# JonasFrey96/Visual-Odom-Pipeline

Measured on AMD Instinct MI355X. Metric: frames/sec @1241x376, 2000 KLT pts, 10-frame BA window, higher is better.
Workload: dtype u8/i32 (KLT, Shi-Tomasi) + f64 (DLT, BA); 1 GPU; kitti_shaped_1241x376_2000pts_ba10; sequences_per_gpu=256, batched_contexts_per_gpu=1, distinct_image_sequences=8, tracked_points=jittered grid (SURVEY 8d's fallback), launch=plain, solves_stopped_by_cap=0, solves_cut_and_rerun=0

## Files before the change

visual-odom-pipeline_amd/csrc/vo_frame.hip:

```cpp
#include "vo_internal.h"

#include <stdlib.h>
#include <string.h>

#include <new>

__device__ __forceinline__ int d_reflect101(int p, int len) {
  if (len == 1) return 0;
  while (p < 0 || p >= len) p = (p < 0) ? -p : 2 * (len - 1) - p;
  return p;
}

struct bil_args {
  int maxk;
  signed char dx[49], dy[49];
  float sw[49];
};

__global__ void __launch_bounds__(256) k_pad_level0_bilateral(const uint8_t* __restrict__ raw, size_t raw_seq_stride,
                                                              const int32_t* __restrict__ frame_idx, int w, int h,
                                                              uint8_t* __restrict__ dst, size_t dst_seq_stride, int pitch,
                                                              int ph, bil_args A, const float* __restrict__ color_w) {
  __shared__ float s_cw[256];
  s_cw[threadIdx.x] = color_w[threadIdx.x];
  __syncthreads();
  const int X = blockIdx.x * blockDim.x + threadIdx.x;
  const int Y = blockIdx.y;
  if (X >= w + 2 * VO_PAD || Y >= ph) return;
  raw += (size_t)blockIdx.z * raw_seq_stride;
  dst += (size_t)blockIdx.z * dst_seq_stride;
  if (frame_idx) raw += (size_t)(*frame_idx) * w * h;
  const int x = d_reflect101(X - VO_PAD, w), y = d_reflect101(Y - VO_PAD, h);
  const int val0 = raw[(size_t)y * w + x];
  float sum = 0.f, wsum = 0.f;
  for (int k = 0; k < A.maxk; k++) {
    const int val = raw[(size_t)d_reflect101(y + A.dy[k], h) * w + d_reflect101(x + A.dx[k], w)];
    const int ad = val > val0 ? val - val0 : val0 - val;
    const float wt = A.sw[k] * s_cw[ad];
    sum += (float)val * wt;
    wsum += wt;
  }
  dst[(size_t)Y * pitch + X] = (uint8_t)(int)__builtin_rintf(sum / wsum);
}

__device__ __forceinline__ bool vo_split_index(unsigned gid, int rows, int gpr, int g_lo, int g_hi, int& Y, int& G) {
  const int gi = g_hi - g_lo, gb = gpr - gi;
  const unsigned n_int = (unsigned)rows * (unsigned)gi;
  if (gid < n_int) {
    Y = (int)(gid / (unsigned)gi);
    G = g_lo + (int)(gid - (unsigned)Y * (unsigned)gi);
    return true;
  }
  gid -= n_int;
  Y = gb > 0 ? (int)(gid / (unsigned)gb) : rows;
  const int j = gb > 0 ? (int)(gid - (unsigned)Y * (unsigned)gb) : 0;
  G = j < g_lo ? j : g_hi + (j - g_lo);
  return false;
}

__global__ void __launch_bounds__(256) k_pad_level0(const uint8_t* __restrict__ raw, size_t raw_seq_stride,
                                                    const int32_t* __restrict__ frame_idx, int w, int h,
                                                    uint8_t* __restrict__ dst, size_t dst_seq_stride, int pitch, int ph, int remap) {
  int blk, bseq;
  vo_xcd_assign(blockIdx.z * gridDim.x + blockIdx.x, gridDim.x, remap, blk, bseq);
  const int gpr = (w + 2 * VO_PAD + 15) / 16;
  const unsigned gid = (unsigned)blk * blockDim.x + threadIdx.x;
  const int g_lo = VO_PAD / 16, g_hi = max(g_lo, min(gpr, (w + VO_PAD - 16 >= 0 ? (w + VO_PAD - 16) / 16 + 1 : 0)));
  int Y, G;
  const bool interior = vo_split_index(gid, ph, gpr, g_lo, g_hi, Y, G);
  const int X = G * 16;
  if (Y >= ph) return;
  raw += (size_t)bseq * raw_seq_stride;
  dst += (size_t)bseq * dst_seq_stride;
  if (frame_idx) raw += (size_t)(*frame_idx) * w * h;
  const int y = d_reflect101(Y - VO_PAD, h);
  const uint8_t* row = raw + (size_t)y * w;
  uint32_t v[4];
  if (interior) {
    __builtin_memcpy(v, row + (X - VO_PAD), 16);
  } else {
#pragma unroll
    for (int q = 0; q < 4; q++) {
      v[q] = 0;
#pragma unroll
      for (int k = 0; k < 4; k++) v[q] |= (uint32_t)row[d_reflect101(X + 4 * q + k - VO_PAD, w)] << (8 * k);
    }
  }
  uint4 pk; pk.x = v[0]; pk.y = v[1]; pk.z = v[2]; pk.w = v[3];
  *reinterpret_cast<uint4*>(dst + (size_t)Y * pitch + X) = pk;
}

__device__ __forceinline__ int d_byte(uint32_t v, int k) { return (int)((v >> (8 * k)) & 0xFFu); }

__global__ void __launch_bounds__(256) k_scharr_pyrdown(const uint8_t* __restrict__ src, size_t src_seq_px, int w, int h, int pitch,
                                                        int16_t* __restrict__ der, int nb_scharr,
                                                        uint8_t* __restrict__ dst, size_t dst_seq_px, int dw, int dh, int dpitch, int remap) {
  int bx, bseq;
  vo_xcd_assign(blockIdx.y * gridDim.x + blockIdx.x, gridDim.x, remap, bx, bseq);
  src += (size_t)bseq * src_seq_px;
  if (bx < nb_scharr) {
    constexpr int SR = 4;
    const int gpr = (w + 3) / 4;
    const unsigned gid = (unsigned)bx * 256u + threadIdx.x;
    const int ys = (int)(gid / (unsigned)gpr);
    const int x0 = (int)(gid - (unsigned)ys * (unsigned)gpr) * 4;
    const int y0 = ys * SR;
    if (y0 >= h) return;
    typedef unsigned short u16x2 __attribute__((ext_vector_type(2)));
    typedef short s16x2 __attribute__((ext_vector_type(2)));
    auto load_row = [&](int yy, u16x2 (&a)[3]) {
      const uint32_t* q = reinterpret_cast<const uint32_t*>(src + (size_t)(yy + VO_PAD) * pitch + (x0 + VO_PAD));
      const uint32_t L = q[-1], M = q[0], R = q[1];
      a[0] = __builtin_bit_cast(u16x2, __builtin_amdgcn_perm(M, L, 0x0c040c03u));
      a[1] = __builtin_bit_cast(u16x2, __builtin_amdgcn_perm(0u, M, 0x0c020c01u));
      a[2] = __builtin_bit_cast(u16x2, __builtin_amdgcn_perm(R, M, 0x0c040c03u));
    };
    u16x2 rows[SR + 2][3];
#pragma unroll
    for (int r = 0; r < SR + 2; r++) load_row(min(y0 - 1 + r, h), rows[r]);
#pragma unroll
    for (int r = 0; r < SR; r++) {
      const int y = y0 + r;
      if (y >= h) break;
      s16x2 cs[3], dv[3];
#pragma unroll
      for (int c = 0; c < 3; c++) {
        cs[c] = __builtin_bit_cast(s16x2, (u16x2)((rows[r][c] + rows[r + 2][c]) * (unsigned short)12 + rows[r + 1][c] * (unsigned short)40));
        dv[c] = __builtin_bit_cast(s16x2, (u16x2)(rows[r + 2][c] - rows[r][c]));
      }
      const uint32_t ix01 = __builtin_bit_cast(uint32_t, (s16x2)(cs[1] - cs[0]));
      const uint32_t ix23 = __builtin_bit_cast(uint32_t, (s16x2)(cs[2] - cs[1]));
      const s16x2 w_lo = {12, 40}, w_hi = {40, 12}, w_0 = {12, 0}, w_1 = {0, 12};
      const int iy0 = __builtin_amdgcn_sdot2(dv[1], w_0, __builtin_amdgcn_sdot2(dv[0], w_lo, 0, false), false);
      const int iy1 = __builtin_amdgcn_sdot2(dv[1], w_hi, __builtin_amdgcn_sdot2(dv[0], w_1, 0, false), false);
      const int iy2 = __builtin_amdgcn_sdot2(dv[2], w_0, __builtin_amdgcn_sdot2(dv[1], w_lo, 0, false), false);
      const int iy3 = __builtin_amdgcn_sdot2(dv[2], w_hi, __builtin_amdgcn_sdot2(dv[1], w_1, 0, false), false);
      uint32_t out[4];
      out[0] = __builtin_amdgcn_perm((uint32_t)iy0, ix01, 0x05040100u);
      out[1] = __builtin_amdgcn_perm((uint32_t)iy1, ix01, 0x05040302u);
      out[2] = __builtin_amdgcn_perm((uint32_t)iy2, ix23, 0x05040100u);
      out[3] = __builtin_amdgcn_perm((uint32_t)iy3, ix23, 0x05040302u);
      if (x0 + 3 >= w) {
#pragma unroll
        for (int k = 1; k < 4; k++) if (x0 + k >= w) out[k] = 0u;
      }
      uint4 pk; pk.x = out[0]; pk.y = out[1]; pk.z = out[2]; pk.w = out[3];
      const size_t o = (size_t)(y + VO_PAD) * pitch + (x0 + VO_PAD);
      *reinterpret_cast<uint4*>(reinterpret_cast<uint32_t*>(der) + (size_t)bseq * src_seq_px + o) = pk;
    }
  } else {
    const int b = bx - nb_scharr;
    const int pw = dw + 2 * VO_PAD;
    const int gpr = (pw + 3) / 4;
    const unsigned gid = (unsigned)b * 256u + threadIdx.x;
    const int g_lo = VO_PAD / 4, g_hi = max(g_lo, min(gpr, (dw + VO_PAD - 4 >= 0 ? (dw + VO_PAD - 4) / 4 + 1 : 0)));
    int Y, G;
    const bool interior = vo_split_index(gid, dh + 2 * VO_PAD, gpr, g_lo, g_hi, Y, G);
    const int X0 = G * 4;
    if (Y >= dh + 2 * VO_PAD) return;
    const int y = d_reflect101(Y - VO_PAD, dh);
    const uint8_t* prow = src + (size_t)(2 * y + VO_PAD) * pitch + VO_PAD;
    uint32_t res = 0;
    if (interior) {
      const int x0 = X0 - VO_PAD;
      uint32_t acc[4] = {128u, 128u, 128u, 128u};
#pragma unroll
      for (int j = -2; j <= 2; j++) {
        const uint32_t* q = reinterpret_cast<const uint32_t*>(prow + (ptrdiff_t)j * pitch + 2 * x0);
        const uint32_t d0 = q[-1], d1 = q[0], d2 = q[1], d3 = q[2];
        const uint32_t wj = (j == 0) ? 6u : ((j == -1 || j == 1) ? 4u : 1u);
        acc[0] = __builtin_amdgcn_udot4(d1, wj * 0x00010406u, __builtin_amdgcn_udot4(d0, wj * 0x04010000u, acc[0], false), false);
        acc[1] = __builtin_amdgcn_udot4(d2, wj * 0x00000001u, __builtin_amdgcn_udot4(d1, wj * 0x04060401u, acc[1], false), false);
        acc[2] = __builtin_amdgcn_udot4(d2, wj * 0x00010406u, __builtin_amdgcn_udot4(d1, wj * 0x04010000u, acc[2], false), false);
        acc[3] = __builtin_amdgcn_udot4(d3, wj * 0x00000001u, __builtin_amdgcn_udot4(d2, wj * 0x04060401u, acc[3], false), false);
      }
      res = __builtin_amdgcn_perm(__builtin_amdgcn_perm(acc[3], acc[2], 0x0c0c0501u), __builtin_amdgcn_perm(acc[1], acc[0], 0x0c0c0501u), 0x05040100u);
    } else {
#pragma unroll
      for (int k = 0; k < 4; k++) {
        const int x = d_reflect101(X0 + k - VO_PAD, dw);
        const uint8_t* p = prow + 2 * x;
        int sum = 0;
#pragma unroll
        for (int j = -2; j <= 2; j++) {
          const uint8_t* r = p + (ptrdiff_t)j * pitch;
          const int row = r[-2] + 4 * r[-1] + 6 * r[0] + 4 * r[1] + r[2];
          const int wj = (j == 0) ? 6 : ((j == -1 || j == 1) ? 4 : 1);
          sum += wj * row;
        }
        res |= (uint32_t)((sum + 128) >> 8) << (8 * k);
      }
    }
    *reinterpret_cast<uint32_t*>(dst + (size_t)bseq * dst_seq_px + (size_t)Y * dpitch + X0) = res;
  }
}

static hipEvent_t prof_event(vo_ctx* c) {
  vo_prof& p = c->prof;
  if (p.used == p.pool.size()) {
    hipEvent_t e = nullptr;
    if (hipEventCreate(&e) != hipSuccess) return nullptr;
    p.pool.push_back(e);
  }
  return p.pool[p.used++];
}

vo_prof_scope::vo_prof_scope(vo_ctx* c_, hipStream_t q_, int region_) : c(c_), q(q_), region(region_) {
  if (!((c->prof.mask >> region) & 1)) return;
  e0 = prof_event(c); e1 = prof_event(c);
  if (e0) (void)hipEventRecord(e0, q);
}

vo_prof_scope::~vo_prof_scope() {
  if (!e0 || !e1) return;
  (void)hipEventRecord(e1, q);
  c->prof.pairs[region].push_back(std::make_pair(e0, e1));
}

extern "C" int32_t vo_profile_enable(vo_ctx* c, int32_t region_mask) {
  if (!c) return VO_E_INVALID;
  VO_HIP(c, hipSetDevice(c->device));
  VO_HIP(c, hipStreamSynchronize(c->stream));
  c->prof.mask = region_mask;
  c->prof.used = 0;
  for (int r = 0; r < VO_PROF_COUNT; r++) c->prof.pairs[r].clear();
  return VO_OK;
}

extern "C" int32_t vo_debug_cycles(vo_ctx* c, int32_t which, int64_t* out8) {
  if (!c) return VO_E_INVALID;
  VO_CHECK(c, which >= 0 && which < 4 && out8, VO_E_INVALID, "bad selector");
  VO_HIP(c, hipSetDevice(c->device));
  VO_HIP(c, hipStreamSynchronize(c->stream));
  unsigned long long h[8];
  VO_HIP(c, hipMemcpy(h, c->d_dbg + 8 * which, sizeof(h), hipMemcpyDeviceToHost));
  out8[0] = 0;
  for (int i = 1; i < 8; i++) out8[i] = (h[i] && h[i - 1] && !(which == 0 && i >= 5)) ? (int64_t)(h[i] - h[i - 1]) : 0;
  for (int i = 1; i < 8; i++) out8[0] += out8[i];
  if (which == 0) { out8[7] = (int64_t)h[6]; out8[5] = (h[5] && h[2]) ? (int64_t)(h[5] - h[2]) : 0; }
  return VO_OK;
}

extern "C" int32_t vo_profile_read(vo_ctx* c, int32_t region, double* total_ms, int32_t* count) {
  if (!c) return VO_E_INVALID;
  VO_CHECK(c, region >= 0 && region < VO_PROF_COUNT && total_ms && count, VO_E_INVALID, "bad region");
  VO_HIP(c, hipSetDevice(c->device));
  VO_HIP(c, hipStreamSynchronize(c->stream));
  double t = 0;
  for (auto& pr : c->prof.pairs[region]) {
    float ms = 0;
    VO_HIP(c, hipEventElapsedTime(&ms, pr.first, pr.second));
    t += ms;
  }
  *total_ms = t; *count = (int32_t)c->prof.pairs[region].size();
  return VO_OK;
}

extern "C" int32_t vo_abi_version(void) { return VO_ABI_VERSION; }

bool vo_blocking_sync() {
  static const bool on = getenv("VO_BLOCKING_SYNC") && atoi(getenv("VO_BLOCKING_SYNC")) != 0;
  return on;
}

extern "C" int32_t vo_device_count(int32_t* n) {
  if (!n) return VO_E_INVALID;
  int c = 0;
  if (hipGetDeviceCount(&c) != hipSuccess) { *n = 0; return VO_E_HIP; }
  *n = c;
  return VO_OK;
}

static thread_local std::string g_create_err;

extern "C" const char* vo_last_error(const vo_ctx* ctx) {
  return ctx ? ctx->err.c_str() : g_create_err.c_str();
}

extern "C" int32_t vo_ctx_destroy(vo_ctx* c) {
  if (!c) return VO_OK;
  (void)hipSetDevice(c->device);
  if (c->stream) (void)hipStreamSynchronize(c->stream);
  if (c->stream2) (void)hipStreamSynchronize(c->stream2);
  if (c->stream_h2d) (void)hipStreamSynchronize(c->stream_h2d);
  if (c->stream3) (void)hipStreamSynchronize(c->stream3);
  (void)vo_comm_destroy(c);
  vo_pipe_destroy(c);
  vo_trk_destroy(c);
  vo_pnp_destroy(c);
  vo_ess_destroy(c);
  vo_hom_destroy(c);
  vo_fund_destroy(c);
  vo_hpose_destroy(c);
  vo_match_destroy(c);
  vo_sift_destroy(c);
  vo_st_destroy(c);
  vo_ba_destroy(c);
  vo_fb_destroy(c);
  vo_guess_destroy(c);
  vo_subpix_destroy(c);
  vo_brief_destroy(c);
  vo_orb_destroy(c);
  vo_ingest_free(&c->und_on, &c->d_und, (void**)&c->d_und_tab);
  vo_ingest_free(&c->cl_on, &c->d_clahe, (void**)&c->d_clahe_lut);
  for (int f = 0; f < 2; f++)
    for (int l = 0; l < VO_MAX_LEVELS; l++) {
      if (c->fr[f].img[l]) (void)hipFree(c->fr[f].img[l]);
      if (c->fr[f].der[l]) (void)hipFree(c->fr[f].der[l]);
    }
  for (auto& g : c->step_graphs) if (g.second) (void)hipGraphExecDestroy(g.second);
  void* bufs[] = {c->d_bil_cw, c->d_dbg, c->d_raw, c->d_seq, c->d_iters, c->d_uv0, c->d_uv1, c->d_slab, c->d_frame_idx, c->d_dlt_cam};
  for (void* b : bufs) if (b) (void)hipFree(b);
  if (c->h_slab) (void)hipHostFree(c->h_slab);
  if (c->h_frame_idx) (void)hipHostFree(c->h_frame_idx);
  if (c->h_raw) (void)hipHostFree(c->h_raw);
  if (c->ev_raw) (void)hipEventDestroy(c->ev_raw);
  for (hipEvent_t e : c->prof.pool) (void)hipEventDestroy(e);
  for (int k = 0; k < 2; k++) if (c->ev_step[k]) (void)hipEventDestroy(c->ev_step[k]);
  if (c->ev_fork) (void)hipEventDestroy(c->ev_fork);
  if (c->ev_join) (void)hipEventDestroy(c->ev_join);
  if (c->stream2) (void)hipStreamDestroy(c->stream2);
  if (c->stream3) (void)hipStreamDestroy(c->stream3);
  for (int k = 0; k < 2; k++) {
    if (c->d_host_raw[k]) (void)hipFree(c->d_host_raw[k]);
    if (c->ev_h2d[k]) (void)hipEventDestroy(c->ev_h2d[k]);
    if (c->ev_raw_free[k]) (void)hipEventDestroy(c->ev_raw_free[k]);
  }
  if (c->stream_h2d) (void)hipStreamDestroy(c->stream_h2d);
  if (c->h_ptr_tab) (void)hipHostFree(c->h_ptr_tab);
  for (int k = 0; k < 2; k++) if (c->ev_ba_wide[k]) (void)hipEventDestroy(c->ev_ba_wide[k]);
  for (int k = 0; k < 2; k++) { if (c->ev_ba[k]) (void)hipEventDestroy(c->ev_ba[k]); if (c->ev_pub[k]) (void)hipEventDestroy(c->ev_pub[k]); if (c->ev_copy1[k]) (void)hipEventDestroy(c->ev_copy1[k]); }
  if (c->stream) (void)hipStreamDestroy(c->stream);
  delete c;
  return VO_OK;
}

hipError_t vo_stream_create(hipStream_t* st, int reserve_cus) {
  int dev = 0, n_cu = 0;
  if (reserve_cus > 0 && (hipGetDevice(&dev) != hipSuccess || hipDeviceGetAttribute(&n_cu, hipDeviceAttributeMultiprocessorCount, dev) != hipSuccess)) n_cu = 0;
  if (reserve_cus <= 0 || n_cu <= 2 * reserve_cus || n_cu > 1024) return hipStreamCreateWithFlags(st, hipStreamNonBlocking);
  uint32_t mask[32];
  for (int k = 0; k < 32; k++) mask[k] = 0;
  for (int b = 0; b < n_cu - reserve_cus; b++) mask[b >> 5] |= 1u << (b & 31);
  return hipExtStreamCreateWithCUMask(st, (uint32_t)((n_cu + 31) / 32), mask);
}

extern "C" int32_t vo_ctx_create(int32_t device, int32_t width, int32_t height, int32_t max_pts,
                                 int32_t max_level, int32_t win, vo_ctx** out) {
  return vo_ctx_create_batched(device, width, height, max_pts, max_level, win, 1, out);
}

extern "C" int32_t vo_ctx_create_batched(int32_t device, int32_t width, int32_t height, int32_t max_pts,
                                         int32_t max_level, int32_t win, int32_t batch, vo_ctx** out) {
  if (!out) return VO_E_INVALID;
  *out = nullptr;
  if (width < 7 || height < 7 || max_pts < 1 || max_level < 0 || max_level >= VO_MAX_LEVELS ||
      win < 3 || win > VO_MAX_WIN || (win & 1) == 0 || batch < 1 || batch > 1024) {
    g_create_err = "vo_ctx_create: invalid argument";
    return VO_E_INVALID;
  }
  int ndev = 0;
  if (hipGetDeviceCount(&ndev) != hipSuccess || ndev <= 0) {
    g_create_err = "vo_ctx_create: no HIP device (this library has no CPU fallback)";
    return VO_E_HIP;
  }
  if (device < 0 || device >= ndev) { g_create_err = "vo_ctx_create: bad device index"; return VO_E_INVALID; }
  vo_ctx* c = new (std::nothrow) vo_ctx();
  if (!c) return VO_E_NOMEM;
  for (int f = 0; f < 2; f++)
    for (int l = 0; l < VO_MAX_LEVELS; l++) { c->fr[f].img[l] = nullptr; c->fr[f].der[l] = nullptr; }
  c->device = device; c->width = width; c->height = height; c->max_pts = max_pts; c->batch = batch;
  c->max_level = max_level; c->win = win;
  auto fail = [&](int32_t code) { g_create_err = c->err; vo_ctx_destroy(c); return code; };
#define CR(expr) do { hipError_t _e = (expr); if (_e != hipSuccess) { c->err = std::string(#expr) + " -> " + hipGetErrorString(_e); return fail(VO_E_HIP); } } while (0)
  CR(hipSetDevice(device));
  CR(hipStreamCreateWithFlags(&c->stream, hipStreamNonBlocking));
  CR(hipStreamCreateWithFlags(&c->stream2, hipStreamNonBlocking));

  CR(hipEventCreateWithFlags(&c->ev_fork, hipEventDisableTiming));
  CR(hipEventCreateWithFlags(&c->ev_join, hipEventDisableTiming));
  {
    const unsigned fl = hipEventDisableTiming | (vo_blocking_sync() ? hipEventBlockingSync : 0u);
    CR(hipEventCreateWithFlags(&c->ev_step[0], fl));
    CR(hipEventCreateWithFlags(&c->ev_step[1], fl));
  }
  int w = width, h = height, top = 0;
  for (int l = 0; l <= max_level; l++) {
    if (l > 0) {
      const int nw = (w + 1) / 2, nh = (h + 1) / 2;
      if (nw <= win || nh <= win) break;
      w = nw; h = nh;
    }
    c->lv[l].w = w; c->lv[l].h = h;
    c->lv[l].pitch = ((w + 2 * VO_PAD + 63) / 64) * 64;
    c->lv[l].ph = h + 2 * VO_PAD;
    c->lvl_px[l] = (size_t)c->lv[l].pitch * c->lv[l].ph;
    top = l;
  }
  c->top = top;
  for (int f = 0; f < 2; f++)
    for (int l = 0; l <= top; l++) {
      const size_t px = c->lvl_px[l] * (size_t)batch;
      CR(hipMalloc((void**)&c->fr[f].img[l], px));
      CR(hipMalloc((void**)&c->fr[f].der[l], px * 4));
      CR(hipMemsetAsync(c->fr[f].img[l], 0, px, c->stream));
      CR(hipMemsetAsync(c->fr[f].der[l], 0, px * 4, c->stream));
    }
  CR(hipMalloc((void**)&c->d_raw, (size_t)width * height * batch));
  CR(hipMalloc((void**)&c->d_dbg, sizeof(unsigned long long) * 32));
  CR(hipMemsetAsync(c->d_dbg, 0, sizeof(unsigned long long) * 32, c->stream));
  {
    size_t off = 0;
    auto take = [&](size_t bytes) { const size_t o = off; off = (off + bytes + 255) & ~(size_t)255; return o; };
    const size_t M = (size_t)max_pts;
    c->off_pa = take(8 * M); c->off_pb = take(8 * M); c->off_status = take(M); c->off_err = take(4 * M);
    c->off_X4 = take(16 * M); c->off_depth = take(8 * M); c->off_reproj = take(8 * M);
    c->off_st_scalars = take(64); c->off_st_out = take(8 * 4096);
    c->slab_seq = off;
    c->slab_bytes = off * (size_t)batch;
    CR(hipMalloc((void**)&c->d_slab, c->slab_bytes));
    CR(hipMemsetAsync(c->d_slab, 0, c->slab_bytes, c->stream));
    CR(hipHostMalloc((void**)&c->h_slab, 2 * c->slab_bytes, hipHostMallocDefault));
  }
  CR(hipMalloc((void**)&c->d_iters, sizeof(int32_t) * (size_t)max_pts * VO_MAX_LEVELS * batch));
  CR(hipMalloc((void**)&c->d_uv0, sizeof(float) * 2 * (size_t)max_pts * batch));
  CR(hipMalloc((void**)&c->d_uv1, sizeof(float) * 2 * (size_t)max_pts * batch));
  CR(hipMalloc((void**)&c->d_frame_idx, sizeof(int32_t)));
  CR(hipHostMalloc((void**)&c->h_frame_idx, sizeof(int32_t) * 64, hipHostMallocDefault));
  CR(hipStreamSynchronize(c->stream));
#undef CR
  *out = c;
  return VO_OK;
}

extern "C" int32_t vo_sync(vo_ctx* c) {
  if (!c) return VO_E_INVALID;
  VO_HIP(c, hipSetDevice(c->device));
  { const int32_t rs = vo_sync_streams(c); if (rs != VO_OK) return rs; }
  if (c->stream_h2d) VO_HIP(c, hipStreamSynchronize(c->stream_h2d));
  return VO_OK;
}

int32_t vo_ingest_reserve(vo_ctx* c, uint8_t** staging) {
  if (!*staging) VO_HIP(c, hipMalloc((void**)staging, (size_t)c->width * c->height * c->batch));
  return VO_OK;
}

int32_t vo_ingest_commit(vo_ctx* c, bool* on) {
  VO_HIP(c, hipStreamSynchronize(c->stream));
  *on = true;
  c->ingest_gen++;
  return VO_OK;
}

void vo_ingest_free(bool* on, uint8_t** staging, void** table) {
  if (*staging) (void)hipFree(*staging);
  if (*table) (void)hipFree(*table);
  *staging = nullptr; *table = nullptr; *on = false;
}

int32_t vo_ingest_run(vo_ctx* c, const vo_ingest_stage& s, const char* off_msg, const uint8_t* img, int32_t stride, uint8_t* out) {
  VO_CHECK(c, img != nullptr && out != nullptr && stride >= c->width, VO_E_INVALID, "bad image / stride");
  VO_CHECK(c, s.on, VO_E_STATE, off_msg);
  VO_HIP(c, hipSetDevice(c->device));
  { const int32_t rq = vo_quiesce_side(c); if (rq != VO_OK) return rq; }
  const size_t rows = (size_t)c->height * c->batch, px = (size_t)c->width * c->height;
  VO_HIP(c, hipMemcpy2DAsync(c->d_raw, c->width, img, stride, c->width, rows, hipMemcpyHostToDevice, c->stream));
  s.enqueue(c, c->stream, c->d_raw, px, nullptr, 0);
  VO_HIP(c, hipGetLastError());
  VO_HIP(c, hipMemcpyAsync(out, s.staging, px * (size_t)c->batch, hipMemcpyDeviceToHost, c->stream));
  VO_HIP(c, hipStreamSynchronize(c->stream));
  return VO_OK;
}

int32_t vo_build_pyramid(vo_ctx* c, hipStream_t q, const uint8_t* d_raw_img, size_t raw_seq_stride, const int32_t* d_frame_idx) {
  vo_prof_scope prof(c, q, VO_PROF_FRAME);
  c->cur ^= 1;
  vo_frame& F = c->fr[c->cur];
  const int B = c->batch;
  const int remap = (!c->tune.xcd_remap_off && B % 8 == 0) ? 1 : 0;
  const vo_ingest_stage chain[2] = {{c->und_on, vo_undistort_enqueue, c->d_und}, {c->cl_on, vo_clahe_enqueue, c->d_clahe}};
  for (const vo_ingest_stage& s : chain)
    if (s.on) {
      s.enqueue(c, q, d_raw_img, raw_seq_stride, d_frame_idx, remap);
      d_raw_img = s.staging; raw_seq_stride = (size_t)c->width * c->height; d_frame_idx = nullptr;
    }
  {
    const vo_level& L = c->lv[0];
    dim3 grid(vo_div_up(((L.w + 2 * VO_PAD + 15) / 16) * L.ph, 256), 1, B);
    dim3 grid1(vo_div_up(L.w + 2 * VO_PAD, 256), L.ph, B);
    if (c->bil_maxk > 0) {
      bil_args A;
      A.maxk = c->bil_maxk;
      for (int k = 0; k < 49; k++) { A.dx[k] = c->bil_dx[k]; A.dy[k] = c->bil_dy[k]; A.sw[k] = c->bil_sw[k]; }
      hipLaunchKernelGGL(k_pad_level0_bilateral, grid1, dim3(256), 0, q, d_raw_img, raw_seq_stride, d_frame_idx, L.w,
                         L.h, F.img[0], c->lvl_px[0], L.pitch, L.ph, A, c->d_bil_cw);
    } else {
      hipLaunchKernelGGL(k_pad_level0, grid, dim3(256), 0, q, d_raw_img, raw_seq_stride, d_frame_idx, L.w, L.h,
                         F.img[0], c->lvl_px[0], L.pitch, L.ph, remap);
    }
  }
  for (int l = 0; l <= c->top; l++) {
    const vo_level& L = c->lv[l];
    const int nb_scharr = vo_div_up(vo_div_up(L.w, 4) * vo_div_up(L.h, 4), 256);
    int nb_down = 0;
    uint8_t* dst = nullptr; int dw = 0, dh = 0, dpitch = 0; size_t dpx = 0;
    if (l < c->top) {
      const vo_level& D = c->lv[l + 1];
      dst = F.img[l + 1]; dw = D.w; dh = D.h; dpitch = D.pitch; dpx = c->lvl_px[l + 1];
      nb_down = vo_div_up(vo_div_up(D.w + 2 * VO_PAD, 4) * D.ph, 256);
    }
    hipLaunchKernelGGL(k_scharr_pyrdown, dim3(nb_scharr + nb_down, B), dim3(256), 0, q,
                       F.img[l], c->lvl_px[l], L.w, L.h, L.pitch, F.der[l], nb_scharr, dst, dpx, dw, dh, dpitch, remap);
  }
  VO_HIP(c, hipGetLastError());
  c->n_pushed++;
  return VO_OK;
}

extern "C" int32_t vo_frame_push(vo_ctx* c, const uint8_t* img, int32_t stride) {
  if (!c) return VO_E_INVALID;
  VO_CHECK(c, img != nullptr && stride >= c->width, VO_E_INVALID, "bad image / stride");
  VO_HIP(c, hipSetDevice(c->device));
  { const int32_t rq = vo_quiesce_side(c); if (rq != VO_OK) return rq; }
  const size_t rows = (size_t)c->height * c->batch, bytes = rows * c->width;
  if (!c->h_raw) {
    VO_HIP(c, hipHostMalloc((void**)&c->h_raw, bytes, hipHostMallocDefault));
    VO_HIP(c, hipEventCreateWithFlags(&c->ev_raw, hipEventDisableTiming));
  } else {
    VO_HIP(c, hipEventSynchronize(c->ev_raw));
  }
  if (stride == c->width) memcpy(c->h_raw, img, bytes);
  else for (size_t y = 0; y < rows; y++) memcpy(c->h_raw + y * c->width, img + y * (size_t)stride, c->width);
  VO_HIP(c, hipMemcpyAsync(c->d_raw, c->h_raw, bytes, hipMemcpyHostToDevice, c->stream));
  VO_HIP(c, hipEventRecord(c->ev_raw, c->stream));
  return vo_build_pyramid(c, c->stream, c->d_raw, (size_t)c->width * c->height, nullptr);
}

extern "C" int32_t vo_seq_upload(vo_ctx* c, const uint8_t* frames, int32_t n_frames) {
  if (!c) return VO_E_INVALID;
  VO_CHECK(c, frames != nullptr && n_frames > 0, VO_E_INVALID, "bad sequence");
  VO_HIP(c, hipSetDevice(c->device));
  { const int32_t rs = vo_sync_streams(c); if (rs != VO_OK) return rs; }
  if (c->d_seq) { VO_HIP(c, hipFree(c->d_seq)); c->d_seq = nullptr; c->seq_n = 0; }
  const size_t bytes = (size_t)c->width * c->height * n_frames * c->batch;
  VO_HIP(c, hipMalloc((void**)&c->d_seq, bytes));
  VO_HIP(c, hipMemcpy(c->d_seq, frames, bytes, hipMemcpyHostToDevice));
  c->seq_n = n_frames;
  return VO_OK;
}

extern "C" int32_t vo_frame_push_resident(vo_ctx* c, int32_t idx) {
  if (!c) return VO_E_INVALID;
  VO_CHECK(c, c->d_seq != nullptr && idx >= 0 && idx < c->seq_n, VO_E_STATE, "no resident sequence / bad index");
  VO_HIP(c, hipSetDevice(c->device));
  { const int32_t rq = vo_quiesce_side(c); if (rq != VO_OK) return rq; }
  const size_t fr = (size_t)c->width * c->height;
  return vo_build_pyramid(c, c->stream, c->d_seq + (size_t)idx * fr, fr * c->seq_n, nullptr);
}

extern "C" int32_t vo_pyramid_level_size(vo_ctx* c, int32_t level, int32_t* w, int32_t* h) {
  if (!c) return VO_E_INVALID;
  VO_CHECK(c, level >= 0 && level <= c->top && w && h, VO_E_INVALID, "bad level");
  *w = c->lv[level].w; *h = c->lv[level].h;
  return VO_OK;
}

extern "C" int32_t vo_pyramid_read(vo_ctx* c, int32_t which, int32_t level, uint8_t* img_out, int16_t* deriv_out) {
  return vo_pyramid_read_seq(c, 0, which, level, img_out, deriv_out);
}

extern "C" int32_t vo_pyramid_read_seq(vo_ctx* c, int32_t seq, int32_t which, int32_t level, uint8_t* img_out, int16_t* deriv_out) {
  if (!c) return VO_E_INVALID;
  VO_CHECK(c, level >= 0 && level <= c->top && (which == 0 || which == 1) && seq >= 0 && seq < c->batch, VO_E_INVALID, "bad level / which / seq");
  VO_CHECK(c, c->n_pushed >= (which == 0 ? 2 : 1), VO_E_STATE, "frame not pushed yet");
  VO_HIP(c, hipSetDevice(c->device));
  const vo_frame& F = c->fr[which == 1 ? c->cur : (c->cur ^ 1)];
  const vo_level& L = c->lv[level];
  VO_HIP(c, hipStreamSynchronize(c->stream));
  if (img_out)
    VO_HIP(c, hipMemcpy2D(img_out, L.w, F.img[level] + (size_t)seq * c->lvl_px[level] + (size_t)VO_PAD * L.pitch + VO_PAD, L.pitch, L.w, L.h,
                          hipMemcpyDeviceToHost));
  if (deriv_out)
    VO_HIP(c, hipMemcpy2D(deriv_out, (size_t)L.w * 4, F.der[level] + ((size_t)seq * c->lvl_px[level] + (size_t)VO_PAD * L.pitch + VO_PAD) * 2,
                          (size_t)L.pitch * 4, (size_t)L.w * 4, L.h, hipMemcpyDeviceToHost));
  if (deriv_out)
    for (size_t i = 0, n = (size_t)L.w * L.h * 2; i < n; i++) deriv_out[i] = (int16_t)(deriv_out[i] / 4);
  return VO_OK;
}

extern "C" int32_t vo_set_prefilter(vo_ctx* c, int32_t d, double sigma_color, double sigma_space) {
  if (!c) return VO_E_INVALID;
  if (d == 0) { c->bil_maxk = 0; c->ingest_gen++; return VO_OK; }
  if (sigma_color <= 0) sigma_color = 1;
  if (sigma_space <= 0) sigma_space = 1;
  int radius = d < 0 ? (int)lrint(sigma_space * 1.5) : d / 2;
  if (radius < 1) radius = 1;
  VO_CHECK(c, radius <= 3, VO_E_CAPACITY, "bilateral pre-filter: diameter up to 7");
  VO_HIP(c, hipSetDevice(c->device));
  const double gc = -0.5 / (sigma_color * sigma_color), gs = -0.5 / (sigma_space * sigma_space);
  float cw[256];
  for (int i = 0; i < 256; i++) cw[i] = (float)exp((double)i * i * gc);
  int maxk = 0;
  for (int i = -radius; i <= radius; i++)
    for (int j = -radius; j <= radius; j++) {
      const double r = sqrt((double)i * i + (double)j * j);
      if (r > radius) continue;
      c->bil_sw[maxk] = (float)exp(r * r * gs);
      c->bil_dx[maxk] = (signed char)j; c->bil_dy[maxk] = (signed char)i;
      maxk++;
    }
  if (!c->d_bil_cw) VO_HIP(c, hipMalloc((void**)&c->d_bil_cw, sizeof(cw)));
  VO_HIP(c, hipMemcpyAsync(c->d_bil_cw, cw, sizeof(cw), hipMemcpyHostToDevice, c->stream));
  VO_HIP(c, hipStreamSynchronize(c->stream));
  c->bil_maxk = maxk;
  c->ingest_gen++;
  return VO_OK;
}
```

Measured before the change: 47720 frames/s.

## Walk row strips in Scharr and pyrDown with register rolling and prefetch

```diff
diff --git a/visual-odom-pipeline_amd/csrc/vo_frame.hip b/visual-odom-pipeline_amd/csrc/vo_frame.hip
--- a/visual-odom-pipeline_amd/csrc/vo_frame.hip
+++ b/visual-odom-pipeline_amd/csrc/vo_frame.hip
@@ -90,92 +90,168 @@
   *reinterpret_cast<uint4*>(dst + (size_t)Y * pitch + X) = pk;
 }
 
-__device__ __forceinline__ int d_byte(uint32_t v, int k) { return (int)((v >> (8 * k)) & 0xFFu); }
+constexpr int VO_WALK_ROWS = 4;
+
+constexpr int VO_SCHARR_STRIP = 8, VO_DOWN_STRIP = 2;
+
+__host__ __device__ inline void vo_down_groups(int dw, int& gpr, int& g_lo, int& g_hi) {
+  gpr = (dw + 2 * VO_PAD + 3) / 4;
+  g_lo = VO_PAD / 4;
+  const int hi = (dw + VO_PAD - 4 >= 0 ? (dw + VO_PAD - 4) / 4 + 1 : 0);
+  g_hi = g_lo > (gpr < hi ? gpr : hi) ? g_lo : (gpr < hi ? gpr : hi);
+}
 
 __global__ void __launch_bounds__(256) k_scharr_pyrdown(const uint8_t* __restrict__ src, size_t src_seq_px, int w, int h, int pitch,
-                                                        int16_t* __restrict__ der, int nb_scharr,
-                                                        uint8_t* __restrict__ dst, size_t dst_seq_px, int dw, int dh, int dpitch, int remap) {
+                                                        int16_t* __restrict__ der, int nb_scharr, int srows,
+                                                        uint8_t* __restrict__ dst, size_t dst_seq_px, int dw, int dh, int dpitch, int drows, int remap) {
   int bx, bseq;
   vo_xcd_assign(blockIdx.y * gridDim.x + blockIdx.x, gridDim.x, remap, bx, bseq);
   src += (size_t)bseq * src_seq_px;
+  typedef unsigned short u16x2 __attribute__((ext_vector_type(2)));
+  typedef short s16x2 __attribute__((ext_vector_type(2)));
+  typedef uint32_t u32x4 __attribute__((ext_vector_type(4)));
   if (bx < nb_scharr) {
-    constexpr int SR = 4;
+    constexpr int CH = VO_WALK_ROWS;
     const int gpr = (w + 3) / 4;
     const unsigned gid = (unsigned)bx * 256u + threadIdx.x;
     const int ys = (int)(gid / (unsigned)gpr);
     const int x0 = (int)(gid - (unsigned)ys * (unsigned)gpr) * 4;
-    const int y0 = ys * SR;
+    const int y0 = ys * srows;
     if (y0 >= h) return;
-    typedef unsigned short u16x2 __attribute__((ext_vector_type(2)));
-    typedef short s16x2 __attribute__((ext_vector_type(2)));
-    auto load_row = [&](int yy, u16x2 (&a)[3]) {
-      const uint32_t* q = reinterpret_cast<const uint32_t*>(src + (size_t)(yy + VO_PAD) * pitch + (x0 + VO_PAD));
-      const uint32_t L = q[-1], M = q[0], R = q[1];
-      a[0] = __builtin_bit_cast(u16x2, __builtin_amdgcn_perm(M, L, 0x0c040c03u));
-      a[1] = __builtin_bit_cast(u16x2, __builtin_amdgcn_perm(0u, M, 0x0c020c01u));
-      a[2] = __builtin_bit_cast(u16x2, __builtin_amdgcn_perm(R, M, 0x0c040c03u));
+    const int y1 = min(y0 + srows, h);
+    const uint8_t* col = src + (size_t)VO_PAD * pitch + (x0 + VO_PAD);
+    auto fetch = [&](int yy, uint32_t (&d)[3]) {
+      const uint32_t* q = reinterpret_cast<const uint32_t*>(col + (ptrdiff_t)min(yy, h) * pitch);
+      d[0] = q[-1]; d[1] = q[0]; d[2] = q[1];
     };
-    u16x2 rows[SR + 2][3];
-#pragma unroll
-    for (int r = 0; r < SR + 2; r++) load_row(min(y0 - 1 + r, h), rows[r]);
-#pragma unroll
-    for (int r = 0; r < SR; r++) {
-      const int y = y0 + r;
-      if (y >= h) break;
-      s16x2 cs[3], dv[3];
-#pragma unroll
-      for (int c = 0; c < 3; c++) {
-        cs[c] = __builtin_bit_cast(s16x2, (u16x2)((rows[r][c] + rows[r + 2][c]) * (unsigned short)12 + rows[r + 1][c] * (unsigned short)40));
-        dv[c] = __builtin_bit_cast(s16x2, (u16x2)(rows[r + 2][c] - rows[r][c]));
+    auto unpack = [&](const uint32_t (&d)[3], u16x2 (&a)[3]) {
+      a[0] = __builtin_bit_cast(u16x2, __builtin_amdgcn_perm(d[1], d[0], 0x0c040c03u));
+      a[1] = __builtin_bit_cast(u16x2, __builtin_amdgcn_perm(0u, d[1], 0x0c020c01u));
+      a[2] = __builtin_bit_cast(u16x2, __builtin_amdgcn_perm(d[2], d[1], 0x0c040c03u));
+    };
+    uint32_t raw[CH][3];
+    u16x2 rows[CH + 2][3];
+    {
+      uint32_t top[2][3];
+      fetch(y0 - 1, top[0]); fetch(y0, top[1]);
+#pragma unroll
+      for (int r = 0; r < CH; r++) fetch(y0 + 1 + r, raw[r]);
+      unpack(top[0], rows[0]); unpack(top[1], rows[1]);
+    }
+    uint32_t* out_px = reinterpret_cast<uint32_t*>(der) + (size_t)bseq * src_seq_px + (size_t)VO_PAD * pitch + (x0 + VO_PAD);
+    for (int y = y0; y < y1; y += CH) {
+#pragma unroll
+      for (int r = 0; r < CH; r++) unpack(raw[r], rows[r + 2]);
+      if (y + CH < y1) {
+#pragma unroll
+        for (int r = 0; r < CH; r++) fetch(y + CH + 1 + r, raw[r]);
       }
-      const uint32_t ix01 = __builtin_bit_cast(uint32_t, (s16x2)(cs[1] - cs[0]));
-      const uint32_t ix23 = __builtin_bit_cast(uint32_t, (s16x2)(cs[2] - cs[1]));
-      const s16x2 w_lo = {12, 40}, w_hi = {40, 12}, w_0 = {12, 0}, w_1 = {0, 12};
-      const int iy0 = __builtin_amdgcn_sdot2(dv[1], w_0, __builtin_amdgcn_sdot2(dv[0], w_lo, 0, false), false);
-      const int iy1 = __builtin_amdgcn_sdot2(dv[1], w_hi, __builtin_amdgcn_sdot2(dv[0], w_1, 0, false), false);
-      const int iy2 = __builtin_amdgcn_sdot2(dv[2], w_0, __builtin_amdgcn_sdot2(dv[1], w_lo, 0, false), false);
-      const int iy3 = __builtin_amdgcn_sdot2(dv[2], w_hi, __builtin_amdgcn_sdot2(dv[1], w_1, 0, false), false);
-      uint32_t out[4];
-      out[0] = __builtin_amdgcn_perm((uint32_t)iy0, ix01, 0x05040100u);
-      out[1] = __builtin_amdgcn_perm((uint32_t)iy1, ix01, 0x05040302u);
-      out[2] = __builtin_amdgcn_perm((uint32_t)iy2, ix23, 0x05040100u);
-      out[3] = __builtin_amdgcn_perm((uint32_t)iy3, ix23, 0x05040302u);
-      if (x0 + 3 >= w) {
-#pragma unroll
-        for (int k = 1; k < 4; k++) if (x0 + k >= w) out[k] = 0u;
+#pragma unroll
+      for (int r = 0; r < CH; r++) {
+        if (y + r >= y1) break;
+        s16x2 cs[3], dv[3];
+#pragma unroll
+        for (int c = 0; c < 3; c++) {
+          cs[c] = __builtin_bit_cast(s16x2, (u16x2)((rows[r][c] + rows[r + 2][c]) * (unsigned short)12 + rows[r + 1][c] * (unsigned short)40));
+          dv[c] = __builtin_bit_cast(s16x2, (u16x2)(rows[r + 2][c] - rows[r][c]));
+        }
+        const uint32_t ix01 = __builtin_bit_cast(uint32_t, (s16x2)(cs[1] - cs[0]));
+        const uint32_t ix23 = __builtin_bit_cast(uint32_t, (s16x2)(cs[2] - cs[1]));
+        const s16x2 w_lo = {12, 40}, w_hi = {40, 12}, w_0 = {12, 0}, w_1 = {0, 12};
+        const int iy0 = __builtin_amdgcn_sdot2(dv[1], w_0, __builtin_amdgcn_sdot2(dv[0], w_lo, 0, false), false);
+        const int iy1 = __builtin_amdgcn_sdot2(dv[1], w_hi, __builtin_amdgcn_sdot2(dv[0], w_1, 0, false), false);
+        const int iy2 = __builtin_amdgcn_sdot2(dv[2], w_0, __builtin_amdgcn_sdot2(dv[1], w_lo, 0, false), false);
+        const int iy3 = __builtin_amdgcn_sdot2(dv[2], w_hi, __builtin_amdgcn_sdot2(dv[1], w_1, 0, false), false);
+        uint32_t out[4];
+        out[0] = __builtin_amdgcn_perm((uint32_t)iy0, ix01, 0x05040100u);
+        out[1] = __builtin_amdgcn_perm((uint32_t)iy1, ix01, 0x05040302u);
+        out[2] = __builtin_amdgcn_perm((uint32_t)iy2, ix23, 0x05040100u);
+        out[3] = __builtin_amdgcn_perm((uint32_t)iy3, ix23, 0x05040302u);
+        if (x0 + 3 >= w) {
+#pragma unroll
+          for (int k = 1; k < 4; k++) if (x0 + k >= w) out[k] = 0u;
+        }
+        const u32x4 pk = {out[0], out[1], out[2], out[3]};
+        __builtin_nontemporal_store(pk, reinterpret_cast<u32x4*>(out_px + (size_t)(y + r) * pitch));
       }
-      uint4 pk; pk.x = out[0]; pk.y = out[1]; pk.z = out[2]; pk.w = out[3];
-      const size_t o = (size_t)(y + VO_PAD) * pitch + (x0 + VO_PAD);
-      *reinterpret_cast<uint4*>(reinterpret_cast<uint32_t*>(der) + (size_t)bseq * src_seq_px + o) = pk;
+#pragma unroll
+      for (int c = 0; c < 3; c++) { rows[0][c] = rows[CH][c]; rows[1][c] = rows[CH + 1][c]; }
     }
   } else {
     const int b = bx - nb_scharr;
-    const int pw = dw + 2 * VO_PAD;
-    const int gpr = (pw + 3) / 4;
-    const unsigned gid = (unsigned)b * 256u + threadIdx.x;
-    const int g_lo = VO_PAD / 4, g_hi = max(g_lo, min(gpr, (dw + VO_PAD - 4 >= 0 ? (dw + VO_PAD - 4) / 4 + 1 : 0)));
+    int gpr, g_lo, g_hi;
+    vo_down_groups(dw, gpr, g_lo, g_hi);
+    const int ph = dh + 2 * VO_PAD, nstrips = (dh + drows - 1) / drows;
+    unsigned gid = (unsigned)b * 256u + threadIdx.x;
+    const uint8_t* pcol = src + (size_t)VO_PAD * pitch + VO_PAD;
+    dst += (size_t)bseq * dst_seq_px;
     int Y, G;
-    const bool interior = vo_split_index(gid, dh + 2 * VO_PAD, gpr, g_lo, g_hi, Y, G);
-    const int X0 = G * 4;
-    if (Y >= dh + 2 * VO_PAD) return;
-    const int y = d_reflect101(Y - VO_PAD, dh);
-    const uint8_t* prow = src + (size_t)(2 * y + VO_PAD) * pitch + VO_PAD;
-    uint32_t res = 0;
-    if (interior) {
-      const int x0 = X0 - VO_PAD;
-      uint32_t acc[4] = {128u, 128u, 128u, 128u};
-#pragma unroll
-      for (int j = -2; j <= 2; j++) {
-        const uint32_t* q = reinterpret_cast<const uint32_t*>(prow + (ptrdiff_t)j * pitch + 2 * x0);
-        const uint32_t d0 = q[-1], d1 = q[0], d2 = q[1], d3 = q[2];
-        const uint32_t wj = (j == 0) ? 6u : ((j == -1 || j == 1) ? 4u : 1u);
-        acc[0] = __builtin_amdgcn_udot4(d1, wj * 0x00010406u, __builtin_amdgcn_udot4(d0, wj * 0x04010000u, acc[0], false), false);
-        acc[1] = __builtin_amdgcn_udot4(d2, wj * 0x00000001u, __builtin_amdgcn_udot4(d1, wj * 0x04060401u, acc[1], false), false);
-        acc[2] = __builtin_amdgcn_udot4(d2, wj * 0x00010406u, __builtin_amdgcn_udot4(d1, wj * 0x04010000u, acc[2], false), false);
-        acc[3] = __builtin_amdgcn_udot4(d3, wj * 0x00000001u, __builtin_amdgcn_udot4(d2, wj * 0x04060401u, acc[3], false), false);
+    if (vo_split_index(gid, nstrips, gpr, g_lo, g_hi, Y, G)) {
+      const int x0 = G * 4 - VO_PAD;
+      const int y0 = Y * drows, y1 = min(y0 + drows, dh);
+      const uint8_t* pc = pcol + 2 * x0;
+      auto fetch = [&](int sy, uint32_t (&d)[4]) {
+        const uint32_t* q = reinterpret_cast<const uint32_t*>(pc + (ptrdiff_t)min(sy, 2 * dh) * pitch);
+        d[0] = q[-1]; d[1] = q[0]; d[2] = q[1]; d[3] = q[2];
+      };
+      auto hpass = [&](const uint32_t (&d)[4], u16x2 (&p)[2]) {
+        const uint32_t h0 = __builtin_amdgcn_udot4(d[1], 0x00010406u, __builtin_amdgcn_udot4(d[0], 0x04010000u, 0u, false), false);
+        const uint32_t h1 = __builtin_amdgcn_udot4(d[2], 0x00000001u, __builtin_amdgcn_udot4(d[1], 0x04060401u, 0u, false), false);
+        const uint32_t h2 = __builtin_amdgcn_udot4(d[2], 0x00010406u, __builtin_amdgcn_udot4(d[1], 0x04010000u, 0u, false), false);
+        const uint32_t h3 = __builtin_amdgcn_udot4(d[3], 0x00000001u, __builtin_amdgcn_udot4(d[2], 0x04060401u, 0u, false), false);
+        p[0] = __builtin_bit_cast(u16x2, h0 | (h1 << 16));
+        p[1] = __builtin_bit_cast(u16x2, h2 | (h3 << 16));
+      };
+      const int P = 2 * (dh - 1);
+      uint32_t raw[4][4];
+      u16x2 em[2], e0[2], om[2];
+      {
+        uint32_t top[3][4];
+        fetch(2 * y0 - 2, top[0]); fetch(2 * y0 - 1, top[1]); fetch(2 * y0, top[2]);
+#pragma unroll
+        for (int r = 0; r < 4; r++) fetch(2 * y0 + 1 + r, raw[r]);
+        hpass(top[0], em); hpass(top[1], om); hpass(top[2], e0);
       }
-      res = __builtin_amdgcn_perm(__builtin_amdgcn_perm(acc[3], acc[2], 0x0c0c0501u), __builtin_amdgcn_perm(acc[1], acc[0], 0x0c0c0501u), 0x05040100u);
+      for (int y = y0; y < y1; y += 2) {
+        u16x2 hp[4][2];
+#pragma unroll
+        for (int r = 0; r < 4; r++) hpass(raw[r], hp[r]);
+        if (y + 2 < y1) {
+#pragma unroll
+          for (int r = 0; r < 4; r++) fetch(2 * y + 5 + r, raw[r]);
+        }
+#pragma unroll
+        for (int r = 0; r < 2; r++) {
+          if (y + r >= y1) break;
+          const u16x2* a = r == 0 ? em : e0;
+          const u16x2* bq = r == 0 ? om : hp[0];
+          const u16x2* c = r == 0 ? e0 : hp[1];
+          const u16x2* d = r == 0 ? hp[0] : hp[2];
+          const u16x2* e = r == 0 ? hp[1] : hp[3];
+          uint32_t s[2];
+#pragma unroll
+          for (int k = 0; k < 2; k++)
+            s[k] = __builtin_bit_cast(uint32_t, (u16x2)((bq[k] + d[k]) * (unsigned short)4 + (c[k] * (unsigned short)6 + (a[k] + e[k])) + (unsigned short)128));
+          const uint32_t res = __builtin_amdgcn_perm(s[1], s[0], 0x07050301u);
+          const int yy = y + r;
+          for (int sgn = 1; sgn >= -1; sgn -= 2) {
+            if (sgn < 0 && (yy == 0 || yy == dh - 1)) break;
+            int p = sgn * yy;
+            while (p - P >= -VO_PAD) p -= P;
+            while (p < -VO_PAD) p += P;
+            for (; p < dh + VO_PAD; p += P) *reinterpret_cast<uint32_t*>(dst + (size_t)(p + VO_PAD) * dpitch + G * 4) = res;
+          }
+        }
+#pragma unroll
+        for (int k = 0; k < 2; k++) { em[k] = hp[1][k]; om[k] = hp[2][k]; e0[k] = hp[3][k]; }
+      }
     } else {
+      gid -= (unsigned)nstrips * (unsigned)(g_hi - g_lo);
+      vo_split_index(gid + (unsigned)ph * (unsigned)(g_hi - g_lo), ph, gpr, g_lo, g_hi, Y, G);
+      if (Y >= ph) return;
+      const int X0 = G * 4;
+      const uint8_t* prow = pcol + (size_t)(2 * d_reflect101(Y - VO_PAD, dh)) * pitch;
+      uint32_t res = 0;
 #pragma unroll
       for (int k = 0; k < 4; k++) {
         const int x = d_reflect101(X0 + k - VO_PAD, dw);
@@ -190,8 +266,8 @@
         }
         res |= (uint32_t)((sum + 128) >> 8) << (8 * k);
       }
-    }
-    *reinterpret_cast<uint32_t*>(dst + (size_t)bseq * dst_seq_px + (size_t)Y * dpitch + X0) = res;
+      *reinterpret_cast<uint32_t*>(dst + (size_t)Y * dpitch + X0) = res;
+    }
   }
 }
 
@@ -502,16 +578,20 @@
   }
   for (int l = 0; l <= c->top; l++) {
     const vo_level& L = c->lv[l];
-    const int nb_scharr = vo_div_up(vo_div_up(L.w, 4) * vo_div_up(L.h, 4), 256);
-    int nb_down = 0;
+    const int srows = VO_SCHARR_STRIP;
+    const int nb_scharr = vo_div_up(vo_div_up(L.w, 4) * vo_div_up(L.h, srows), 256);
+    int nb_down = 0, drows = 0;
     uint8_t* dst = nullptr; int dw = 0, dh = 0, dpitch = 0; size_t dpx = 0;
     if (l < c->top) {
       const vo_level& D = c->lv[l + 1];
       dst = F.img[l + 1]; dw = D.w; dh = D.h; dpitch = D.pitch; dpx = c->lvl_px[l + 1];
-      nb_down = vo_div_up(vo_div_up(D.w + 2 * VO_PAD, 4) * D.ph, 256);
+      drows = VO_DOWN_STRIP;
+      int gpr, g_lo, g_hi;
+      vo_down_groups(D.w, gpr, g_lo, g_hi);
+      nb_down = vo_div_up((g_hi - g_lo) * vo_div_up(D.h, drows) + (gpr - (g_hi - g_lo)) * D.ph, 256);
     }
     hipLaunchKernelGGL(k_scharr_pyrdown, dim3(nb_scharr + nb_down, B), dim3(256), 0, q,
-                       F.img[l], c->lvl_px[l], L.w, L.h, L.pitch, F.der[l], nb_scharr, dst, dpx, dw, dh, dpitch, remap);
+                       F.img[l], c->lvl_px[l], L.w, L.h, L.pitch, F.der[l], nb_scharr, srows, dst, dpx, dw, dh, dpitch, drows, remap);
   }
   VO_HIP(c, hipGetLastError());
   c->n_pushed++;
```

Result: faster. 48410 frames/s (median of 5 runs) (+1.4%).
